# cvg/nice-slam

Hardware: NVIDIA H100
Metric: rendered rays/sec (higher is better)
Workload: dtype f32

## Files before the change

### nice_slam_b200/csrc/nsb_tc.cuh

```cuda
#pragma once

namespace nsb {
namespace tc {

#ifdef NSB_PHASE_TIMING
__device__ long long g_phase[64];
__device__ long long g_phase_last;
#define NSB_PH(id) do { if (blockIdx.x == 0 && threadIdx.x == 0) { const long long c_ = clock64(); ::nsb::tc::g_phase[id] += c_ - ::nsb::tc::g_phase_last; ::nsb::tc::g_phase_last = c_; } } while (0)
#define NSB_PH_RESET() do { if (blockIdx.x == 0 && threadIdx.x == 0) ::nsb::tc::g_phase_last = clock64(); } while (0)
#else
#define NSB_PH(id) do { } while (0)
#define NSB_PH_RESET() do { } while (0)
#endif

constexpr int TM = 128;
constexpr int kThreads = 512;
constexpr int kCG = kThreads / TM;
constexpr int kCW = 32 / kCG;
constexpr int kKQ = kCW / 4;

__device__ __forceinline__ float to_tf32(float x) { return __uint_as_float(__float_as_uint(x) & 0xffffe000u); }

__device__ __forceinline__ int canon_q(int r, int kq, int K) { return ((r >> 3) * (K >> 2) + kq) * 32 + (r & 7) * 4; }

// ... 11 lines not shown
  d |= (uint64_t)((smem_u32(smem) >> 4) & 0x3FFF);
  d |= (uint64_t)((lbo_bytes >> 4) & 0x3FFF) << 16;
  d |= (uint64_t)((sbo_bytes >> 4) & 0x3FFF) << 32;
  return d;
}

constexpr int kAccCols = 256;
constexpr int kAccSlotsPerSm = 4;
constexpr int kAccMaxSm = 144;
__device__ float g_acc_pool[(size_t)kAccMaxSm * kAccSlotsPerSm * kAccCols * TM];
__device__ int g_acc_lock[kAccMaxSm * kAccSlotsPerSm];
__shared__ float* s_acc;
__device__ __forceinline__ uint32_t acc_acquire() {
  uint32_t smid;
  asm volatile("mov.u32 %0, %%smid;" : "=r"(smid));
  if (smid >= (uint32_t)kAccMaxSm) __trap();
  const long long t0 = clock64();
  for (;;) {
    for (int k = 0; k < kAccSlotsPerSm; k++) {
      const int s = (int)smid * kAccSlotsPerSm + k;
      if (atomicCAS(&g_acc_lock[s], 0, 1) == 0) {
        __threadfence();
        s_acc = g_acc_pool + (size_t)s * kAccCols * TM;
        return (uint32_t)s;
      }
    }
    if (clock64() - t0 > 4000000000ll) __trap();
  }
}
__device__ __forceinline__ void acc_release(uint32_t slot) { __threadfence(); atomicExch(&g_acc_lock[slot], 0); }
__device__ __forceinline__ const float* acc_col(uint32_t taddr) { return s_acc + (size_t)(taddr & 0xffffu) * TM + (taddr >> 16) + (threadIdx.x & 31); }

__device__ __forceinline__ void wg_fence() { asm volatile("wgmma.fence.sync.aligned;" ::: "memory"); }
__device__ __forceinline__ void wg_commit_wait() {
  asm volatile("wgmma.commit_group.sync.aligned;" ::: "memory");
  asm volatile("wgmma.wait_group.sync.aligned 0;" ::: "memory");
}
__device__ __forceinline__ void wg_commit() { asm volatile("wgmma.commit_group.sync.aligned;" ::: "memory"); }
__device__ __forceinline__ void wg_wait0() { asm volatile("wgmma.wait_group.sync.aligned 0;" ::: "memory"); }
template <int N>
__device__ __forceinline__ void wg_wait() { asm volatile("wgmma.wait_group.sync.aligned %0;" ::"n"(N) : "memory"); }
__device__ __forceinline__ void fence_acc(float (&d)[16]) {
#pragma unroll
  for (int e = 0; e < 16; e++) asm volatile("" : "+f"(d[e])::"memory");
}
#define NSB_WG_D16 "+f"(d[0]), "+f"(d[1]), "+f"(d[2]), "+f"(d[3]), "+f"(d[4]), "+f"(d[5]), "+f"(d[6]), "+f"(d[7]), \
                   "+f"(d[8]), "+f"(d[9]), "+f"(d[10]), "+f"(d[11]), "+f"(d[12]), "+f"(d[13]), "+f"(d[14]), "+f"(d[15])
__device__ __forceinline__ void wgmma_tf32_n32(float (&d)[16], uint64_t da, uint64_t db) {
  asm volatile("{\n\t.reg .pred p;\n\tsetp.ne.b32 p, 1, 0;\n\t"
               "wgmma.mma_async.sync.aligned.m64n32k8.f32.tf32.tf32 "
               "{%0,%1,%2,%3,%4,%5,%6,%7,%8,%9,%10,%11,%12,%13,%14,%15}, %16, %17, p, 1, 1;\n\t}"
               : NSB_WG_D16 : "l"(da), "l"(db));
}
__device__ __forceinline__ void wgmma_f16_n32(float (&d)[16], uint64_t da, uint64_t db) {
  asm volatile("{\n\t.reg .pred p;\n\tsetp.ne.b32 p, 1, 0;\n\t"
               "wgmma.mma_async.sync.aligned.m64n32k16.f32.f16.f16 "
               "{%0,%1,%2,%3,%4,%5,%6,%7,%8,%9,%10,%11,%12,%13,%14,%15}, %16, %17, p, 1, 1, 0, 0;\n\t}"
               : NSB_WG_D16 : "l"(da), "l"(db));
}
#define NSB_WG_D32 "+f"(d0[0]), "+f"(d0[1]), "+f"(d0[2]), "+f"(d0[3]), "+f"(d0[4]), "+f"(d0[5]), "+f"(d0[6]), "+f"(d0[7]), \
                   "+f"(d0[8]), "+f"(d0[9]), "+f"(d0[10]), "+f"(d0[11]), "+f"(d0[12]), "+f"(d0[13]), "+f"(d0[14]), "+f"(d0[15]), \
                   "+f"(d1[0]), "+f"(d1[1]), "+f"(d1[2]), "+f"(d1[3]), "+f"(d1[4]), "+f"(d1[5]), "+f"(d1[6]), "+f"(d1[7]), \
                   "+f"(d1[8]), "+f"(d1[9]), "+f"(d1[10]), "+f"(d1[11]), "+f"(d1[12]), "+f"(d1[13]), "+f"(d1[14]), "+f"(d1[15])
#define NSB_WG_R32 "{%0,%1,%2,%3,%4,%5,%6,%7,%8,%9,%10,%11,%12,%13,%14,%15,%16,%17,%18,%19,%20,%21,%22,%23,%24,%25,%26,%27,%28,%29,%30,%31}"
__device__ __forceinline__ void wgmma_tf32_n64(float (&d0)[16], float (&d1)[16], uint64_t da, uint64_t db) {
  asm volatile("{\n\t.reg .pred p;\n\tsetp.ne.b32 p, 1, 0;\n\t"
               "wgmma.mma_async.sync.aligned.m64n64k8.f32.tf32.tf32 " NSB_WG_R32 ", %32, %33, p, 1, 1;\n\t}"
               : NSB_WG_D32 : "l"(da), "l"(db));
}
__device__ __forceinline__ void wgmma_f16_n64(float (&d0)[16], float (&d1)[16], uint64_t da, uint64_t db) {
  asm volatile("{\n\t.reg .pred p;\n\tsetp.ne.b32 p, 1, 0;\n\t"
               "wgmma.mma_async.sync.aligned.m64n64k16.f32.f16.f16 " NSB_WG_R32 ", %32, %33, p, 1, 1, 0, 0;\n\t}"
               : NSB_WG_D32 : "l"(da), "l"(db));
}
__device__ __forceinline__ void frag_rc(int e, int& r, int& c) {
  const int l = threadIdx.x & 31, w = (threadIdx.x >> 5) & 3;
  r = 16 * w + (l >> 2) + 8 * ((e >> 1) & 1);
  c = 8 * (e >> 2) + 2 * (l & 3) + (e & 1);
}

template <bool H16>
__device__ __forceinline__ void wg_mma(uint32_t dcol, uint64_t ah, uint64_t al, uint32_t sboA, uint64_t bh, uint64_t bl, uint32_t sboB,
                                       int N, int ksteps, uint32_t acc) {
  const int wg = threadIdx.x >> 7, npairs = blockDim.x >> 8;
  const int rbase = 64 * (wg & 1);
  const uint64_t aoff = (uint64_t)((8u * sboA * (uint32_t)(wg & 1)) >> 4);
  for (int c = wg >> 1; c < (N >> 5); c += npairs) {
    float* base = s_acc + (size_t)(dcol + 32 * c) * TM + rbase;
    float d[16];
#pragma unroll
    for (int e = 0; e < 16; e++) { int r, cc; frag_rc(e, r, cc); d[e] = acc ? base[cc * TM + r] : 0.0f; }
    const uint64_t boff = (uint64_t)((4u * sboB * (uint32_t)c) >> 4);
    wg_fence();
#pragma unroll 1
    for (int ks = 0; ks < ksteps; ks++) {
      const uint64_t o = 16u * (uint64_t)ks;
      if (H16) {
        wgmma_f16_n32(d, al + aoff + o, bh + boff + o); wgmma_f16_n32(d, ah + aoff + o, bl + boff + o); wgmma_f16_n32(d, ah + aoff + o, bh + boff + o);
      } else {
        wgmma_tf32_n32(d, al + aoff + o, bh + boff + o); wgmma_tf32_n32(d, ah + aoff + o, bl + boff + o); wgmma_tf32_n32(d, ah + aoff + o, bh + boff + o);
      }
    }
    wg_commit_wait();
#pragma unroll
    for (int e = 0; e < 16; e++) { int r, cc; frag_rc(e, r, cc); base[cc * TM + r] = d[e]; }
  }
}
__device__ __forceinline__ void mbar_arrive1(uint64_t* bar) { asm volatile("mbarrier.arrive.shared::cta.b64 _, [%0];" ::"r"(smem_u32(bar)) : "memory"); }
__device__ __forceinline__ void group_done(uint64_t* bar) {
  __syncthreads();
  if (threadIdx.x == 0) mbar_arrive1(bar);
}
__device__ __forceinline__ void mma_3x(uint32_t d_tmem, const float* a_hi, const float* a_lo, int KA, int ka0,
                                       const float* b_hi, const float* b_lo, int KB, int kb0, int kcount, int N, uint32_t& acc) {
  const uint32_t sboA = (uint32_t)(KA >> 2) * 128u, sboB = (uint32_t)(KB >> 2) * 128u;
  const uint64_t ah0 = make_desc(a_hi + (ka0 >> 2) * 32, 128u, sboA), al0 = make_desc(a_lo + (ka0 >> 2) * 32, 128u, sboA);
  const uint64_t bh0 = make_desc(b_hi + (kb0 >> 2) * 32, 128u, sboB), bl0 = make_desc(b_lo + (kb0 >> 2) * 32, 128u, sboB);
  wg_mma<false>(d_tmem & 0xffffu, ah0, al0, sboA, bh0, bl0, sboB, N, kcount, acc);
  acc = 1u;
}
__device__ __forceinline__ void publish_operands() { fence_proxy_async(); __syncthreads(); }

__device__ __forceinline__ void acc_ld8(uint32_t taddr, float (&v)[8]) {
  const float* p = acc_col(taddr);
#pragma unroll
  for (int j = 0; j < 8; j++) v[j] = p[j * TM];
}
static_assert(kCW == 8, "epilogues read 8 accumulator columns per thread");

struct TcSmem {
  float* x;
// ... 355 lines not shown
```

### nice_slam_b200/csrc/nsb_tile.cuh

```cuda
#pragma once

namespace nsb {
namespace tl {

using tc::TM;
constexpr int kThreads = 256;
constexpr int kEpiThreads = kThreads;
constexpr int kCG = 2, kCW = 16, kKQ = 4;
constexpr int kSlots = 4;
constexpr int kSlotFloatsFwd = 2560;
constexpr int kSlotFloatsBwd = 2048;
constexpr int kABufFloats = 2 * TM * 32;
constexpr int kMaxTileRays = 18;
constexpr int kMinSamples = 8;
constexpr long long kWaitCycles = 4000000000ll;

enum { B_FULL = 0, B_EMPTY = 4, B_HDR = 8, B_AREADY = 10, B_DONE = 12, kNumBars = 14 };

__device__ __forceinline__ bool mbar_try(uint64_t* bar, uint32_t parity) {
  uint32_t ok;
  asm volatile("{\n\t.reg .pred p;\n\tmbarrier.try_wait.parity.shared::cta.b64 p, [%1], %2;\n\tselp.b32 %0, 1, 0, p;\n\t}"
               : "=r"(ok) : "r"(smem_u32(bar)), "r"(parity) : "memory");
  return ok != 0;
}
// ... 95 lines not shown
  uint32_t issued;
  uint32_t g;
};
__device__ __forceinline__ void issuer_wait_operands(Issuer& I, const TileSmem& t, int b, uint32_t parity) {
  uint64_t* bar = t.bars + B_AREADY + b;
  const long long t0 = clock64();
  while (!mbar_test(bar, parity)) {
    if (threadIdx.x == 0) loader_top_up(I.L, t, I.issued);
    if (clock64() - t0 > kWaitCycles) __trap();
  }
}
__device__ __forceinline__ const float* issuer_unit(Issuer& I, const TileSmem& t, uint32_t k = 0) {
  if (threadIdx.x == 0) {
    loader_top_up(I.L, t, I.issued);
    while (I.L.loaded <= I.issued + k) loader_refill(I.L, t, I.issued);
  }
  const uint32_t u = I.issued + k;
  const int slot = u & (kSlots - 1);
  mbar_wait_b(t.bars + B_FULL + slot, (u >> 2) & 1u);
  return t.ring + slot * t.slot_floats;
}
__device__ __forceinline__ const float* issued_unit(const Issuer& I, const TileSmem& t, uint32_t k) { return t.ring + ((I.issued + k) & (kSlots - 1)) * t.slot_floats; }

__device__ __forceinline__ uint32_t cvt_h2(float lo_elem, float hi_elem) {
  uint32_t r;
  asm("cvt.rn.satfinite.f16x2.f32 %0, %1, %2;" : "=r"(r) : "f"(hi_elem), "f"(lo_elem));
  return r;
}
__device__ __forceinline__ void split_h2(float x, float y, uint32_t& h, uint32_t& l) {
  h = cvt_h2(x, y);
  const float2 f = __half22float2(*reinterpret_cast<const __half2*>(&h));
  l = cvt_h2(x - f.x, y - f.y);
}
__device__ __forceinline__ void put4_h(float* tile, int r, int kq, const float4 v) {
  unsigned char* hi = reinterpret_cast<unsigned char*>(tile) + (((r >> 3) * 4 + (kq >> 1)) * 128 + (r & 7) * 16 + (kq & 1) * 8);
  uint2 h, l;
  split_h2(v.x, v.y, h.x, l.x); split_h2(v.z, v.w, h.y, l.y);
  *reinterpret_cast<uint2*>(hi) = h;
  *reinterpret_cast<uint2*>(hi + TM * 32 * 2) = l;
}
__device__ __forceinline__ void put16_h(float* tile, int r, int cg, const float (&v)[kCW]) {
#pragma unroll
  for (int c = 0; c < 2; c++) {
    unsigned char* hi = reinterpret_cast<unsigned char*>(tile) + (((r >> 3) * 4 + 2 * cg + c) * 128 + (r & 7) * 16);
    uint4 h, l;
    split_h2(v[8 * c], v[8 * c + 1], h.x, l.x); split_h2(v[8 * c + 2], v[8 * c + 3], h.y, l.y);
    split_h2(v[8 * c + 4], v[8 * c + 5], h.z, l.z); split_h2(v[8 * c + 6], v[8 * c + 7], h.w, l.w);
    *reinterpret_cast<uint4*>(hi) = h;
    *reinterpret_cast<uint4*>(hi + TM * 32 * 2) = l;
  }
}
struct RowsDesc { uint64_t ah, al, bh, bl; };
template <bool H16>
__device__ __forceinline__ RowsDesc rows_desc(const float* a, int ka0, const float* b, int N, int KB, int c) {
  const uint32_t g = (threadIdx.x >> 7) & 1u;
  const int esz = H16 ? 2 : 4, kcm = H16 ? 8 : 4;
  const uint32_t sbo_a = (32u / kcm) * 128u, sbo_b = (uint32_t)(KB / kcm) * 128u;
  RowsDesc r;
  r.ah = tc::make_desc(a + (ka0 / kcm) * 32, 128u, sbo_a) + (uint64_t)((8u * sbo_a * g) >> 4);
  r.bh = tc::make_desc(b, 128u, sbo_b) + (uint64_t)((4u * sbo_b * (uint32_t)c) >> 4);
  r.al = r.ah + (uint64_t)((TM * 32 * esz) >> 4); r.bl = r.bh + (uint64_t)((N * KB * esz) >> 4);
  return r;
}
template <bool H16, int ksteps>
__device__ __forceinline__ void mma_rows(float (&d)[16], const float* a, int ka0, const float* b, int N, int KB, int c) {
  const RowsDesc r = rows_desc<H16>(a, ka0, b, N, KB, c);
#pragma unroll
  for (int ks = 0; ks < ksteps; ks++) {
    const uint64_t o = 16u * (uint64_t)ks;
    if (H16) { tc::wgmma_f16_n32(d, r.al + o, r.bh + o); tc::wgmma_f16_n32(d, r.ah + o, r.bl + o); tc::wgmma_f16_n32(d, r.ah + o, r.bh + o); }
    else { tc::wgmma_tf32_n32(d, r.al + o, r.bh + o); tc::wgmma_tf32_n32(d, r.ah + o, r.bl + o); tc::wgmma_tf32_n32(d, r.ah + o, r.bh + o); }
  }
}
template <bool H16, int ksteps>
__device__ __forceinline__ void mma_rows64(float (&d0)[16], float (&d1)[16], const float* a, int ka0, const float* b, int N, int KB, int c) {
  const RowsDesc r = rows_desc<H16>(a, ka0, b, N, KB, c);
#pragma unroll
  for (int ks = 0; ks < ksteps; ks++) {
    const uint64_t o = 16u * (uint64_t)ks;
    if (H16) { tc::wgmma_f16_n64(d0, d1, r.al + o, r.bh + o); tc::wgmma_f16_n64(d0, d1, r.ah + o, r.bl + o); tc::wgmma_f16_n64(d0, d1, r.ah + o, r.bh + o); }
    else { tc::wgmma_tf32_n64(d0, d1, r.al + o, r.bh + o); tc::wgmma_tf32_n64(d0, d1, r.ah + o, r.bl + o); tc::wgmma_tf32_n64(d0, d1, r.ah + o, r.bh + o); }
  }
}
__device__ __forceinline__ void arrive_units(const TileSmem& t, uint32_t first, uint32_t count, uint64_t* done = nullptr) {
  if ((threadIdx.x & 127) == 0) {
    for (uint32_t k = 0; k < count; k++) mbar_arrive(t.bars + B_EMPTY + ((first + k) & (kSlots - 1)));
    if (done != nullptr) mbar_arrive(done);
  }
}
__device__ __forceinline__ void release_units(Issuer& I, const TileSmem& t, uint32_t count, uint64_t* done = nullptr) {
  arrive_units(t, I.issued, count, done);
  I.issued += count;
}
__device__ __forceinline__ void wg_bar_sync() {
  if (threadIdx.x >> 7) asm volatile("bar.sync 2, 128;" ::: "memory");
  else asm volatile("bar.sync 1, 128;" ::: "memory");
}
__device__ __forceinline__ void zero16(float (&d)[16]) {
#pragma unroll
  for (int e = 0; e < 16; e++) d[e] = 0.0f;
}
__device__ __forceinline__ void zero16_opaque(float (&d)[16]) {
#pragma unroll
  for (int e = 0; e < 16; e++) asm volatile("mov.b32 %0, 0;" : "=f"(d[e])::"memory");
}
__device__ __forceinline__ void put2(float* hi, int r, int c, float a, float b) {
  float* hp = hi + tc::canon_q(r, c >> 2, 32) + (c & 3);
  const float h0 = tc::to_tf32(a), h1 = tc::to_tf32(b);
  *reinterpret_cast<float2*>(hp) = make_float2(h0, h1);
  *reinterpret_cast<float2*>(hp + TM * 32) = make_float2(a - h0, b - h1);
}

__device__ __forceinline__ void publish(const TileSmem& t, int b) {
  fence_proxy_async();
  __syncwarp();
  if ((threadIdx.x & 31) == 0) mbar_arrive(t.bars + B_AREADY + b);
}
__device__ __forceinline__ void wait_group(const TileSmem& t, uint32_t m) {
  mbar_wait_b(t.bars + B_DONE + (m & 1u), (m >> 1) & 1u);
}

struct GatherPass {
  float4 v[8];
  float w[8];
// ... 81 lines not shown
#pragma unroll
  for (int k = 0; k < 4; k++) p[k] = make_float4(d[4 * k], d[4 * k + 1], d[4 * k + 2], d[4 * k + 3]);
}
template <bool H16, bool kAccumulate>
__device__ __forceinline__ void issue_fc(Issuer& I, const TileSmem& t, float (&d1)[16], float (&d3)[16]) {
  constexpr int nu = H16 ? 2 : 4;
  const int b = I.g & 1;
  issuer_wait_operands(I, t, b, (I.g >> 1) & 1u);
  NSB_PH(5);
#pragma unroll 1
  for (int u = 0; u < nu; u++) issuer_unit(I, t, u);
  NSB_PH(11);
#pragma unroll
  for (int c = 0; c < 5; c += 2) {
    const bool pair = c < 4;
    if (kAccumulate) { ld_frag(d2_frag(c), d1); if (pair) ld_frag(d2_frag(c + 1), d3); }
    else { zero16_opaque(d1); if (pair) zero16_opaque(d3); }
    tc::wg_fence();
#pragma unroll
    for (int u = 0; u < nu; u++) {
      if (pair) mma_rows64<H16, 1>(d1, d3, t.a[b], H16 ? 16 * u : 8 * u, issued_unit(I, t, u), 160, H16 ? 16 : 8, c);
      else mma_rows<H16, 1>(d1, t.a[b], H16 ? 16 * u : 8 * u, issued_unit(I, t, u), 160, H16 ? 16 : 8, c);
    }
    tc::wg_commit(); tc::wg_wait0(); tc::fence_acc(d1);
    st_frag(d2_frag(c), d1);
    if (pair) { tc::fence_acc(d3); st_frag(d2_frag(c + 1), d3); }
  }
  release_units(I, t, nu, t.bars + B_DONE + b);
  I.g++;
}
template <bool H16 = false>
__device__ __forceinline__ void issue_l0(Issuer& I, const TileSmem& t, float (&d1)[16], float (&d3)[16]) {
  constexpr int nu = H16 ? 1 : 2;
  const int b = I.g & 1;
  issuer_wait_operands(I, t, b, (I.g >> 1) & 1u);
  NSB_PH(10);
#pragma unroll 1
  for (int u = 0; u < nu; u++) issuer_unit(I, t, u);
  tc::wg_fence();
#pragma unroll
  for (int u = 0; u < nu; u++) mma_rows64<H16, 2>(d1, d3, t.a[b], 16 * u, issued_unit(I, t, u), 64, H16 ? 32 : 16, 0);
  tc::wg_commit();
  I.issued += nu;
  I.g++;
}
template <bool H16 = false>
__device__ __forceinline__ void release_l0(const Issuer& I, const TileSmem& t, uint32_t back, uint32_t count) {
  constexpr uint32_t nu = H16 ? 1 : 2;
  for (uint32_t j = back; j > back - count; j--) arrive_units(t, I.issued - j * nu, nu, t.bars + B_DONE + ((I.g - j) & 1u));
}
template <bool H16 = false>
__device__ __forceinline__ void issue_h(Issuer& I, const TileSmem& t, float (&d1)[16], const float (&d3)[16], const float* hbuf, int i) {
  const float* w = issuer_unit(I, t);
  if (i == 3) {
#pragma unroll
    for (int e = 0; e < 16; e++) d1[e] = d3[e];
  } else {
    zero16(d1);
  }
  tc::wg_fence();
  mma_rows<H16, H16 ? 2 : 4>(d1, hbuf, 0, w, 32, 32, 0);
  tc::wg_commit();
}

template <bool H16 = false>
__device__ __forceinline__ void epi_forward(const KParams& P, const TileSmem& t, Issuer& I, int lv, const PointGeom& G, uint32_t& n, int hb, uint32_t hdr_parity,
                                            float (&out)[4], uint32_t* __restrict__ masks, float* __restrict__ acts, int npts) {
  const int row = threadIdx.x & (TM - 1), cg = threadIdx.x >> 7, warp = threadIdx.x >> 5, lane = threadIdx.x & 31;
  const bool xyz = lv != 0;
  const int cd = op_cd(lv), no = lv == 3 ? 4 : 1;
  const float* hdr = t.hdr + hb * kHdrFloats;
  float d1[16], d3[16];
  if (xyz) {
    for (int half = 0; half < cd / 32; half++) {
      if (n >= 2) wait_group(t, n - 2);
      if (threadIdx.x == 0) loader_top_up(I.L, t, I.issued);
      gather_tile<H16>(P.in.grid[half == 0 ? lv : 1], t.a[n & 1], G.xn, warp, lane);
      NSB_PH(1);
      publish(t, n & 1); n++;
      if (half == 0) issue_fc<H16, false>(I, t, d1, d3); else issue_fc<H16, true>(I, t, d1, d3);
      NSB_PH(2);
    }
    mbar_wait_b(t.bars + B_HDR + hb, hdr_parity);
    zero16_opaque(d1); zero16_opaque(d3);
#pragma unroll
    for (int blk = 0; blk < 3; blk++) {
      if (n >= 2) wait_group(t, n - 2);
      if (threadIdx.x == 0) loader_top_up(I.L, t, I.issued);
      NSB_PH(6);
      embed_tile<H16>(t.a[n & 1], hdr + 464, G.pf, row, cg, blk);
      NSB_PH(3);
      publish(t, n & 1); n++;
      issue_l0<H16>(I, t, d1, d3);
      if (blk == 1) { tc::wg_wait<1>(); release_l0<H16>(I, t, 2, 1); }
      NSB_PH(4);
    }
  } else {
    if (n >= 2) wait_group(t, n - 2);
    gather_tile<H16>(P.in.grid[0], t.a[n & 1], G.xnc, warp, lane);
    publish(t, n & 1); n++;
    zero16_opaque(d1); zero16_opaque(d3);
    issue_l0<H16>(I, t, d1, d3);
    mbar_wait_b(t.bars + B_HDR + hb, hdr_parity);
  }
  tc::wg_wait0(); tc::fence_acc(d1); tc::fence_acc(d3);
  release_l0<H16>(I, t, xyz ? 2 : 1, xyz ? 2 : 1);
  st_frag(d2_frag(5), d3);
  float* hbuf = t.a[n & 1];
  const int wg = threadIdx.x >> 7, q = lane & 3;
  const int r0 = 64 * wg + 16 * (warp & 3) + (lane >> 2);
  float v2[16];
  if (xyz) ld_frag(d2_frag(0), v2);
#pragma unroll 1
  for (int i = 0; i < 5; i++) {
    if (threadIdx.x == 0) loader_top_up(I.L, t, I.issued);
    NSB_PH(7);
    uint32_t m0 = 0, m1 = 0;
#pragma unroll
    for (int e = 0; e < 16; e++) {
      const int c = 8 * (e >> 2) + 2 * q + (e & 1);
      const float u = d1[e] + hdr[i * 32 + c];
      const uint32_t bit = u > 0.0f ? 1u << (8 * (e >> 2) + (e & 1)) : 0u;
      if (e & 2) m1 |= bit; else m0 |= bit;
      float h = u > 0.0f ? u : 0.0f;
      if (xyz) h += v2[e] + hdr[160 + i * 32 + c];
      d1[e] = h;
    }
    if (masks != nullptr) {
      m0 <<= 2 * q; m1 <<= 2 * q;
      m0 |= __shfl_xor_sync(0xffffffffu, m0, 1); m1 |= __shfl_xor_sync(0xffffffffu, m1, 1);
      m0 |= __shfl_xor_sync(0xffffffffu, m0, 2); m1 |= __shfl_xor_sync(0xffffffffu, m1, 2);
      if (q == 0 && r0 < npts) masks[(size_t)r0 * 15 + i] = m0;
      if (q == 1 && r0 + 8 < npts) masks[(size_t)(r0 + 8) * 15 + i] = m1;
    }
    if (acts != nullptr) {
#pragma unroll
      for (int e = 0; e < 16; e += 2) {
        const int r = r0 + 8 * ((e >> 1) & 1), c = 8 * (e >> 2) + 2 * q;
        if (r < npts) __stcg(reinterpret_cast<float2*>(acts + (size_t)r * 160 + i * 32 + c), make_float2(d1[e], d1[e + 1]));
      }
    }
    if (i == 4) break;
    if (i == 2) ld_frag(d2_frag(5), d3);
#pragma unroll
    for (int e = 0; e < 16; e += 2) {
      const int r = r0 + 8 * ((e >> 1) & 1), c = 8 * (e >> 2) + 2 * q;
      if (H16) {
        unsigned char* hp = reinterpret_cast<unsigned char*>(hbuf) + (((r >> 3) * 4 + (c >> 3)) * 128 + (r & 7) * 16 + (c & 7) * 2);
        uint32_t hh, ll;
        split_h2(d1[e], d1[e + 1], hh, ll);
        *reinterpret_cast<uint32_t*>(hp) = hh;
        *reinterpret_cast<uint32_t*>(hp + TM * 32 * 2) = ll;
      } else {
        put2(hbuf, r, c, d1[e], d1[e + 1]);
      }
    }
    NSB_PH(8);
    fence_proxy_async();
    wg_bar_sync();
    issue_h<H16>(I, t, d1, d3, hbuf, i + 1);
    NSB_PH(9);
    if (xyz) ld_frag(d2_frag(i + 1), v2);
    tc::wg_wait0(); tc::fence_acc(d1); release_units(I, t, 1);
  }
  NSB_PH(8);
  float s0[4], s1[4];
#pragma unroll
  for (int o = 0; o < 4; o++) {
    s0[o] = s1[o] = 0.0f;
    if (o < no) {
#pragma unroll
      for (int e = 0; e < 16; e++) {
        const float w = hdr[336 + o * 32 + 8 * (e >> 2) + 2 * q + (e & 1)];
        if (e & 2) s1[o] = fmaf(d1[e], w, s1[o]); else s0[o] = fmaf(d1[e], w, s0[o]);
      }
    }
    s0[o] += __shfl_xor_sync(0xffffffffu, s0[o], 1); s1[o] += __shfl_xor_sync(0xffffffffu, s1[o], 1);
    s0[o] += __shfl_xor_sync(0xffffffffu, s0[o], 2); s1[o] += __shfl_xor_sync(0xffffffffu, s1[o], 2);
  }
  constexpr int kWgHiFloats = 64 * 32 / (H16 ? 2 : 1);
  auto part = [&](int r) { return reinterpret_cast<float4*>(hbuf + (r >> 6) * kWgHiFloats + (r & 63) * 4); };
  if (q == 0) *part(r0) = make_float4(s0[0], s0[1], s0[2], s0[3]);
  if (q == 1) *part(r0 + 8) = make_float4(s1[0], s1[1], s1[2], s1[3]);
  epi_sync();
  {
    const float4 v = *part(row);
    out[0] = hdr[320] + v.x; out[1] = hdr[321] + v.y; out[2] = hdr[322] + v.z; out[3] = hdr[323] + v.w;
  }
  epi_sync();
  NSB_PH(12);
}

constexpr int kMnTile = TM * 32;
constexpr size_t kWgBytes = (size_t)6 * kMnTile * 4;
constexpr int kWgALo = 2 * kMnTile, kWgBLo = kMnTile;
struct WgSmem { float* du; float* g; float* b; float* dpk; };
__host__ __device__ __forceinline__ int acts_slot(int mask, int lv) { return (mask >> lv) & 1 ? __builtin_popcount(mask & ((1 << lv) - 1)) : -1; }
struct WgDec { int o_W0, o_W1, o_W2, o_W3E, o_W3H, o_W4, o_WC, PC, o_WO, no, o_b, o_bc, o_bo; };
template <int LV>
__device__ __forceinline__ WgDec wg_dec() {
  using D = Dec<LV>;
  return WgDec{D::o_W0, D::o_W1, D::o_W2, D::o_W3E, D::o_W3H, D::o_W4, D::o_WC, D::PC, D::o_WO, D::NO, D::o_b, D::o_bc, D::o_bo};
}
static_assert(Dec<0>::PH == Dec<3>::PH && Dec<1>::PH == Dec<3>::PH && Dec<2>::PH == Dec<3>::PH, "shared hidden pitch of the WG decoders");
static_assert(Dec<1>::PF == Dec<3>::PF && Dec<2>::PF == Dec<3>::PF && Dec<1>::o_B == Dec<3>::o_B && Dec<2>::o_B == Dec<3>::o_B,
              "shared first-input pitch and embedding block of the xyz WG decoders");
static_assert(Dec<1>::o_WO == Dec<3>::o_WO && Dec<1>::o_bo == Dec<3>::o_bo && Dec<1>::TOTAL == Dec<3>::TOTAL, "middle decoder = colour layout");
__device__ __forceinline__ void split4(const float4 v, float4& h, float4& l) {
  h = make_float4(tc::to_tf32(v.x), tc::to_tf32(v.y), tc::to_tf32(v.z), tc::to_tf32(v.w));
  l = make_float4(v.x - h.x, v.y - h.y, v.z - h.z, v.w - h.w);
}
__device__ __forceinline__ int kt_idx(int f, int p) { return ((f >> 3) * (TM / 4) + (p >> 2)) * 32 + (f & 7) * 4 + (p & 3); }
// ... 63 lines not shown
      }
    }
  }
  __syncthreads();
}
__device__ __forceinline__ float warp_colsum16(const float (&v)[kCW], int lane) {
  float a[8];
#pragma unroll
  for (int j = 0; j < 8; j++) { const float give = (lane & 16) ? v[j] : v[j + 8], keep = (lane & 16) ? v[j + 8] : v[j]; a[j] = keep + __shfl_xor_sync(0xffffffffu, give, 16); }
  float b[4];
#pragma unroll
  for (int j = 0; j < 4; j++) { const float give = (lane & 8) ? a[j] : a[j + 4], keep = (lane & 8) ? a[j + 4] : a[j]; b[j] = keep + __shfl_xor_sync(0xffffffffu, give, 8); }
  float c[2];
#pragma unroll
  for (int j = 0; j < 2; j++) { const float give = (lane & 4) ? b[j] : b[j + 2], keep = (lane & 4) ? b[j + 2] : b[j]; c[j] = keep + __shfl_xor_sync(0xffffffffu, give, 4); }
  const float give = (lane & 2) ? c[0] : c[1], keep = (lane & 2) ? c[1] : c[0];
  float d = keep + __shfl_xor_sync(0xffffffffu, give, 2);
  d += __shfl_xor_sync(0xffffffffu, d, 1);
  return d;
}
__device__ __forceinline__ int colsum_col(int lane) { return ((lane >> 4) & 1) * 8 + ((lane >> 3) & 1) * 4 + ((lane >> 2) & 1) * 2 + ((lane >> 1) & 1); }
__device__ __forceinline__ float frag_colsum(const float (&v)[16], int lane) {
  float a[8];
#pragma unroll
  for (int j = 0; j < 8; j++) a[j] = v[4 * (j >> 1) + (j & 1)] + v[4 * (j >> 1) + (j & 1) + 2];
  float b[4];
#pragma unroll
  for (int j = 0; j < 4; j++) { const float give = (lane & 16) ? a[j] : a[j + 4], keep = (lane & 16) ? a[j + 4] : a[j]; b[j] = keep + __shfl_xor_sync(0xffffffffu, give, 16); }
  float c[2];
#pragma unroll
  for (int j = 0; j < 2; j++) { const float give = (lane & 8) ? b[j] : b[j + 2], keep = (lane & 8) ? b[j + 2] : b[j]; c[j] = keep + __shfl_xor_sync(0xffffffffu, give, 8); }
  const float give = (lane & 4) ? c[0] : c[1], keep = (lane & 4) ? c[1] : c[0];
  return keep + __shfl_xor_sync(0xffffffffu, give, 4);
}
__device__ __forceinline__ int frag_colsum_col(int lane) {
  const int j = ((lane >> 4) & 1) * 4 + ((lane >> 3) & 1) * 2 + ((lane >> 2) & 1);
  return 8 * (j >> 1) + 2 * (lane & 3) + (j & 1);
}

struct BwdExtra {
  double dp[TM * 3];
  double z[TM];
  float gocc[TM];
  float wgt[TM];
  float gc[kMaxTileRays * 3];
};
__device__ __forceinline__ void bwd_gout(const BwdExtra& X, int lv, int r, int npts, int off0, int S, float (&go)[4]) {
  go[0] = go[1] = go[2] = go[3] = 0.0f;
  if (r >= npts) return;
  if (lv == 3) { const float w = X.wgt[r]; const float* gc = X.gc + 3 * ((off0 + r) / S); go[0] = w * gc[0]; go[1] = w * gc[1]; go[2] = w * gc[2]; }
  else go[0] = X.gocc[r];
}

template <bool DC, int NDF, bool L0>
__device__ __forceinline__ void issue_bwd_layer_t(Issuer& I, const TileSmem& t, int ndc, float (&d1)[16], float (&dc)[16], float (&fa)[16]) {
  constexpr int ND1 = L0 ? 0 : 1, FMAX = L0 ? 2 : 1;
  constexpr int kWaves = NDF > FMAX ? (NDF + FMAX - 1) / FMAX : 1;
#pragma unroll
  for (int wave = 0; wave < kWaves; wave++) {
    const int f0 = wave * FMAX;
    const int nf = NDF - f0 < FMAX ? NDF - f0 : FMAX;
    const int k = wave == 0 ? ndc + ND1 : 0;
    const int nu = k + nf;
#pragma unroll 1
    for (int u = 0; u < nu; u++) issuer_unit(I, t, u);
    if (nf > 0) { if (L0) ld_frag(d2_frag(f0), fa); else zero16_opaque(fa); }
    if (nf > 1) ld_frag(d2_frag(f0 + 1), d1);
    if (wave == 0 && ND1) zero16_opaque(d1);
    tc::wg_fence();
    if (wave == 0) {
      if (DC) mma_rows<false, 4>(dc, t.a[0], 0, issued_unit(I, t, 0), 32, 32, 0);
      if (ND1) mma_rows<false, 4>(d1, t.a[1], 0, issued_unit(I, t, ndc), 32, 32, 0);
    }
    if (nf > 0) mma_rows<false, 4>(fa, t.a[1], 0, issued_unit(I, t, k), 32, 32, 0);
    if (nf > 1) mma_rows<false, 4>(d1, t.a[1], 0, issued_unit(I, t, k + 1), 32, 32, 0);
    tc::wg_commit(); tc::wg_wait0();
    tc::fence_acc(dc); tc::fence_acc(d1); tc::fence_acc(fa);
    if (nf > 0) st_frag(d2_frag(f0), fa);
    if (nf > 1) st_frag(d2_frag(f0 + 1), d1);
    release_units(I, t, nu);
  }
}
template <bool XYZ>
__device__ __forceinline__ void issue_bwd_layer_x(Issuer& I, const TileSmem& t, int ndc, int i, float (&d1)[16], float (&dc)[16], float (&fa)[16]) {
  constexpr int NDF = op_firstp(XYZ ? 1 : 0) / 32;
  if (XYZ && i == 4) zero16_opaque(dc);
  if (i == 3) issue_bwd_layer_t<XYZ, NDF, false>(I, t, ndc, d1, dc, fa);
  else if (i == 0) issue_bwd_layer_t<XYZ, NDF, true>(I, t, ndc, d1, dc, fa);
  else issue_bwd_layer_t<XYZ, 0, false>(I, t, ndc, d1, dc, fa);
}
__device__ __forceinline__ void issue_bwd_layer(Issuer& I, const TileSmem& t, int lv, int i, float (&d1)[16], float (&dc)[16], float (&fa)[16]) {
  if (lv != 0) issue_bwd_layer_x<true>(I, t, op_cd(lv) / 32, i, d1, dc, fa);
  else issue_bwd_layer_x<false>(I, t, 0, i, d1, dc, fa);
}

enum { kWgNone = 0, kWgXyz = 1, kWgCoarse = 2 };
__device__ __forceinline__ int bwd_dpe_off(int r) { return (r >> 6) * (64 * 32) + (r & 63) * 4; }
template <int WG>
__device__ __forceinline__ void epi_backward(const KParams& P, const TileSmem& t, Issuer& I, const BwdExtra& X, int lv, const PointGeom& G, int hb, uint32_t hdr_parity,
                                             const uint32_t* __restrict__ masks, int npts, int off0, long long gp0, WgSmem* w = nullptr, const float* acts_row = nullptr) {
  const int row = threadIdx.x & (TM - 1), cg = threadIdx.x >> 7, warp = threadIdx.x >> 5;
  const int lane = threadIdx.x & 31, q = lane & 3;
  const int r0 = 64 * (threadIdx.x >> 7) + 16 * (warp & 3) + (lane >> 2);
  const int S = P.S;
  constexpr bool kWg = WG != kWgNone;
  constexpr int PH = Dec<3>::PH, PF = WG == kWgCoarse ? Dec<0>::PF : Dec<3>::PF;
  const WgDec DW = WG == kWgCoarse ? wg_dec<0>() : lv == 2 ? wg_dec<2>() : wg_dec<3>();
  float creg[kCW], cmid[kCW];
  const bool xyz = WG == kWgCoarse ? false : lv != 0;
  const float* hdr = t.hdr + hb * kHdrFloats;
  uint32_t m01 = 0, m23 = 0, m4 = 0;
  {
    const uint32_t* w0 = masks + (size_t)(r0 < npts ? r0 : npts - 1) * 15;
    const uint32_t* w1 = masks + (size_t)(r0 + 8 < npts ? r0 + 8 : npts - 1) * 15;
#pragma unroll
    for (int i = 0; i < 5; i++) {
      const uint32_t v = ((w0[i] >> (2 * q)) & 0x03030303u) | (((w1[i] >> (2 * q)) & 0x03030303u) << 2);
      if (i == 4) m4 = v; else if (i & 2) m23 |= v << (4 * (i & 1)); else m01 |= v << (4 * (i & 1));
    }
  }
  mbar_wait_b(t.bars + B_HDR + hb, hdr_parity);
  float d1[16], dc[16], fa[16];
  {
    float go0[4], go1[4];
    bwd_gout(X, lv, r0, npts, off0, S, go0); bwd_gout(X, lv, r0 + 8, npts, off0, S, go1);
#pragma unroll
    for (int e = 0; e < 16; e++) {
      float v = 0.0f;
#pragma unroll
      for (int o = 0; o < 4; o++) v = fmaf(hdr[336 + o * 32 + 8 * (e >> 2) + 2 * q + (e & 1)], (e & 2) ? go1[o] : go0[o], v);
      d1[e] = v;
    }
  }
  if constexpr (kWg) {
    float g_out[4];
    bwd_gout(X, lv, row, npts, off0, S, g_out);
    gather_tile_kt(P.in.grid[lv], w->b, kWgBLo, WG == kWgCoarse ? G.xnc : G.xn, warp, lane);
    __syncthreads();
    get_kt16(w->b, kWgBLo, row, cg, creg);
    __syncthreads();
    if (lv == 2) {
      gather_tile_kt(P.in.grid[NSB_MIDDLE], w->b, kWgBLo, G.xn, warp, lane);
      __syncthreads();
      get_kt16(w->b, kWgBLo, row, cg, cmid);
      __syncthreads();
    }
    float go[kCW];
#pragma unroll
    for (int j = 0; j < kCW; j++) go[j] = (cg == 0 && j < 4) ? g_out[j] : 0.0f;
    put_kt16(w->du, kWgALo, row, cg, go);
    float h4[kCW];
#pragma unroll
    for (int k = 0; k < kKQ; k++) {
      const float4 v = acts_row != nullptr ? __ldcg(reinterpret_cast<const float4*>(acts_row + 4 * 32 + 4 * k)) : make_float4(0.f, 0.f, 0.f, 0.f);
      h4[4 * k] = v.x; h4[4 * k + 1] = v.y; h4[4 * k + 2] = v.z; h4[4 * k + 3] = v.w;
    }
    put_kt16(w->b, kWgBLo, row, cg, h4);
    wg_group(*w, 0, w->dpk + DW.o_WO, PH, DW.no);
    if (cg == 0) {
      const float sb = warp_colsum16(go, lane);
      const int col = colsum_col(lane);
      if ((lane & 1) == 0 && col < DW.no) atomicAdd(w->dpk + DW.o_bo + col, sb);
    }
  }
#pragma unroll 1
  for (int i = 4; i >= 0; i--) {
    const uint32_t m = (i == 4 ? m4 : (i & 2) ? m23 : m01) >> (4 * (i & 1));
    float du[16];
#pragma unroll
    for (int e = 0; e < 16; e++) du[e] = (m >> (8 * (e >> 2) + 2 * ((e >> 1) & 1) + (e & 1))) & 1u ? d1[e] : 0.0f;
#pragma unroll
    for (int e = 0; e < 16; e += 2) {
      const int r = r0 + 8 * ((e >> 1) & 1), c = 8 * (e >> 2) + 2 * q;
      if (xyz) put2(t.a[0], r, c, d1[e], d1[e + 1]);
      put2(t.a[1], r, c, du[e], du[e + 1]);
    }
    if constexpr (kWg) {
#pragma unroll
      for (int e = 0; e < 16; e++) {
        const int r = r0 + 8 * ((e >> 1) & 1), c = 8 * (e >> 2) + 2 * q + (e & 1);
        put_kt1(w->du, kWgALo, c, r, du[e]);
        if constexpr (WG != kWgCoarse) put_kt1(w->g, kWgALo, c, r, d1[e]);
      }
      const float sb = frag_colsum(du, lane);
      float sc = 0.0f;
      if constexpr (WG != kWgCoarse) sc = frag_colsum(d1, lane);
      const int col = frag_colsum_col(lane);
      atomicAdd(w->dpk + DW.o_b + 32 * i + col, sb);
      if constexpr (WG != kWgCoarse) atomicAdd(w->dpk + DW.o_bc + 32 * i + col, sc);
    }
    fence_proxy_async();
    wg_bar_sync();
    NSB_PH(22);
    issue_bwd_layer(I, t, WG == kWgCoarse ? 0 : lv, i, d1, dc, fa);
    if (threadIdx.x == 0) loader_top_up(I.L, t, I.issued);
    NSB_PH(23);
    if constexpr (kWg) {
      if (i >= 1) {
        float xr[kCW];
#pragma unroll
        for (int k = 0; k < kKQ; k++) {
          const float4 v = acts_row != nullptr ? __ldcg(reinterpret_cast<const float4*>(acts_row + (i - 1) * 32 + 4 * k)) : make_float4(0.f, 0.f, 0.f, 0.f);
          xr[4 * k] = v.x; xr[4 * k + 1] = v.y; xr[4 * k + 2] = v.z; xr[4 * k + 3] = v.w;
        }
        put_kt16(w->b, kWgBLo, row, cg, xr);
        const int o_wh = i == 1 ? DW.o_W1 : i == 2 ? DW.o_W2 : i == 3 ? DW.o_W3H : DW.o_W4;
        wg_group(*w, 0, w->dpk + o_wh, PH, 32);
      }
      if constexpr (WG != kWgCoarse) {
        put_kt16(w->b, kWgBLo, row, cg, creg);
        wg_group(*w, 1, w->dpk + DW.o_WC + 32 * i * DW.PC, DW.PC, 32);
        if (lv == 2) {
          put_kt16(w->b, kWgBLo, row, cg, cmid);
          wg_group(*w, 1, w->dpk + DW.o_WC + 32 * i * DW.PC + 32, DW.PC, 32);
        }
      }
      if (i == 3 || i == 0) {
        if constexpr (WG != kWgCoarse) {
          const float* B = hdr + 464;
          for (int blk = 0; blk < 3; blk++) {
            float e[kCW];
#pragma unroll
            for (int j = 0; j < kCW; j++) {
              const int f = 32 * blk + kCW * cg + j;
              float x = G.pf[0] * B[f]; x = fmaf(G.pf[1], B[kEmbPad + f], x); x = fmaf(G.pf[2], B[2 * kEmbPad + f], x);
              e[j] = f < kEmb ? __sinf(reduce_2pi(x)) : 0.0f;
            }
            put_kt16(w->b, kWgBLo, row, cg, e);
            wg_group(*w, 0, w->dpk + (i == 0 ? DW.o_W0 : DW.o_W3E) + 32 * blk, PF, 32);
          }
        } else {
          put_kt16(w->b, kWgBLo, row, cg, creg);
          wg_group(*w, 0, w->dpk + (i == 0 ? DW.o_W0 : DW.o_W3E), PF, 32);
        }
      }
      NSB_PH(24);
    }
  }
  if (!xyz) ld_frag(d2_frag(0), dc);
#pragma unroll
  for (int e = 0; e < 16; e += 2) {
    const int r = r0 + 8 * ((e >> 1) & 1), c = 8 * (e >> 2) + 2 * q;
    *reinterpret_cast<float2*>(t.a[0] + r * 32 + c) = make_float2(dc[e], dc[e + 1]);
  }
  float dpe0[3] = {0.0f, 0.0f, 0.0f}, dpe1[3] = {0.0f, 0.0f, 0.0f};
  if (xyz) {
    const float* B = hdr + 464;
// ... 374 lines not shown
```

Before: 1.258 million.

## Feed hidden-layer MMA A operand from registers instead of shared memory

Adds a register-sourced wgmma variant for TF32 and a shuffle-based conversion of the accumulator fragment into the A-operand layout, split into hi/lo TF32 parts. The forward hidden layers and the backward hidden layers without DF chunks now feed activations straight from registers. This skips the shared-memory staging stores, the async-proxy fence and the warpgroup barrier on those paths. In exchange it adds shuffles and register pressure, and the register-fragment permutation must be exactly right for correctness.

```diff
diff --git a/nice_slam_b200/csrc/nsb_tc.cuh b/nice_slam_b200/csrc/nsb_tc.cuh
--- a/nice_slam_b200/csrc/nsb_tc.cuh
+++ b/nice_slam_b200/csrc/nsb_tc.cuh
@@ -87,6 +87,12 @@
                "{%0,%1,%2,%3,%4,%5,%6,%7,%8,%9,%10,%11,%12,%13,%14,%15}, %16, %17, p, 1, 1;\n\t}"
                : NSB_WG_D16 : "l"(da), "l"(db));
 }
+__device__ __forceinline__ void wgmma_tf32_n32_rs(float (&d)[16], const uint32_t (&a)[4], uint64_t db) {
+  asm volatile("{\n\t.reg .pred p;\n\tsetp.ne.b32 p, 1, 0;\n\t"
+               "wgmma.mma_async.sync.aligned.m64n32k8.f32.tf32.tf32 "
+               "{%0,%1,%2,%3,%4,%5,%6,%7,%8,%9,%10,%11,%12,%13,%14,%15}, {%16,%17,%18,%19}, %20, p, 1, 1;\n\t}"
+               : NSB_WG_D16 : "r"(a[0]), "r"(a[1]), "r"(a[2]), "r"(a[3]), "l"(db));
+}
 __device__ __forceinline__ void wgmma_f16_n32(float (&d)[16], uint64_t da, uint64_t db) {
   asm volatile("{\n\t.reg .pred p;\n\tsetp.ne.b32 p, 1, 0;\n\t"
                "wgmma.mma_async.sync.aligned.m64n32k16.f32.f16.f16 "
@@ -112,6 +118,24 @@
   const int l = threadIdx.x & 31, w = (threadIdx.x >> 5) & 3;
   r = 16 * w + (l >> 2) + 8 * ((e >> 1) & 1);
   c = 8 * (e >> 2) + 2 * (l & 3) + (e & 1);
+}
+__device__ __forceinline__ void frag_a_tf32(const float (&d)[16], uint32_t (&ah)[16], uint32_t (&al)[16]) {
+  const int lane = threadIdx.x & 31, q = lane & 3, quad = lane & ~3;
+  const int src1 = quad | ((q & 1) << 1) | (q >> 1), src2 = quad | (((q & 1) ^ 1) << 1) | (q >> 1);
+  const bool upper = (q >> 1) != 0;
+#pragma unroll
+  for (int j = 0; j < 4; j++) {
+#pragma unroll
+    for (int h = 0; h < 2; h++) {
+      const float x0 = d[4 * j + 2 * h], x1 = d[4 * j + 2 * h + 1];
+      const float v1 = __shfl_sync(0xffffffffu, upper ? x1 : x0, src1);
+      const float v2 = __shfl_sync(0xffffffffu, upper ? x0 : x1, src2);
+      const float cq = (q & 1) ? v2 : v1, cq4 = (q & 1) ? v1 : v2;
+      const float hq = to_tf32(cq), hq4 = to_tf32(cq4);
+      ah[4 * j + h] = __float_as_uint(hq); al[4 * j + h] = __float_as_uint(cq - hq);
+      ah[4 * j + 2 + h] = __float_as_uint(hq4); al[4 * j + 2 + h] = __float_as_uint(cq4 - hq4);
+    }
+  }
 }
 
 template <bool H16>
diff --git a/nice_slam_b200/csrc/nsb_tile.cuh b/nice_slam_b200/csrc/nsb_tile.cuh
--- a/nice_slam_b200/csrc/nsb_tile.cuh
+++ b/nice_slam_b200/csrc/nsb_tile.cuh
@@ -171,14 +171,21 @@
 }
 struct RowsDesc { uint64_t ah, al, bh, bl; };
 template <bool H16>
+__device__ __forceinline__ void b_desc(const float* b, int N, int KB, int c, uint64_t& bh, uint64_t& bl) {
+  const int esz = H16 ? 2 : 4, kcm = H16 ? 8 : 4;
+  const uint32_t sbo_b = (uint32_t)(KB / kcm) * 128u;
+  bh = tc::make_desc(b, 128u, sbo_b) + (uint64_t)((4u * sbo_b * (uint32_t)c) >> 4);
+  bl = bh + (uint64_t)((N * KB * esz) >> 4);
+}
+template <bool H16>
 __device__ __forceinline__ RowsDesc rows_desc(const float* a, int ka0, const float* b, int N, int KB, int c) {
   const uint32_t g = (threadIdx.x >> 7) & 1u;
   const int esz = H16 ? 2 : 4, kcm = H16 ? 8 : 4;
-  const uint32_t sbo_a = (32u / kcm) * 128u, sbo_b = (uint32_t)(KB / kcm) * 128u;
+  const uint32_t sbo_a = (32u / kcm) * 128u;
   RowsDesc r;
   r.ah = tc::make_desc(a + (ka0 / kcm) * 32, 128u, sbo_a) + (uint64_t)((8u * sbo_a * g) >> 4);
-  r.bh = tc::make_desc(b, 128u, sbo_b) + (uint64_t)((4u * sbo_b * (uint32_t)c) >> 4);
-  r.al = r.ah + (uint64_t)((TM * 32 * esz) >> 4); r.bl = r.bh + (uint64_t)((N * KB * esz) >> 4);
+  r.al = r.ah + (uint64_t)((TM * 32 * esz) >> 4);
+  b_desc<H16>(b, N, KB, c, r.bh, r.bl);
   return r;
 }
 template <bool H16, int ksteps>
@@ -189,6 +196,18 @@
     const uint64_t o = 16u * (uint64_t)ks;
     if (H16) { tc::wgmma_f16_n32(d, r.al + o, r.bh + o); tc::wgmma_f16_n32(d, r.ah + o, r.bl + o); tc::wgmma_f16_n32(d, r.ah + o, r.bh + o); }
     else { tc::wgmma_tf32_n32(d, r.al + o, r.bh + o); tc::wgmma_tf32_n32(d, r.ah + o, r.bl + o); tc::wgmma_tf32_n32(d, r.ah + o, r.bh + o); }
+  }
+}
+template <int ksteps>
+__device__ __forceinline__ void mma_rows_rs(float (&d)[16], const uint32_t (&ah)[4 * ksteps], const uint32_t (&al)[4 * ksteps], const float* b, int N, int KB, int c) {
+  uint64_t bh, bl;
+  b_desc<false>(b, N, KB, c, bh, bl);
+#pragma unroll
+  for (int ks = 0; ks < ksteps; ks++) {
+    const uint64_t o = 16u * (uint64_t)ks;
+    const uint32_t (&h)[4] = *reinterpret_cast<const uint32_t (*)[4]>(ah + 4 * ks);
+    const uint32_t (&l)[4] = *reinterpret_cast<const uint32_t (*)[4]>(al + 4 * ks);
+    tc::wgmma_tf32_n32_rs(d, l, bh + o); tc::wgmma_tf32_n32_rs(d, h, bl + o); tc::wgmma_tf32_n32_rs(d, h, bh + o);
   }
 }
 template <bool H16, int ksteps>
@@ -376,6 +395,8 @@
 template <bool H16 = false>
 __device__ __forceinline__ void issue_h(Issuer& I, const TileSmem& t, float (&d1)[16], const float (&d3)[16], const float* hbuf, int i) {
   const float* w = issuer_unit(I, t);
+  uint32_t ah[16], al[16];
+  if constexpr (!H16) tc::frag_a_tf32(d1, ah, al);
   if (i == 3) {
 #pragma unroll
     for (int e = 0; e < 16; e++) d1[e] = d3[e];
@@ -383,7 +404,8 @@
     zero16(d1);
   }
   tc::wg_fence();
-  mma_rows<H16, H16 ? 2 : 4>(d1, hbuf, 0, w, 32, 32, 0);
+  if constexpr (H16) mma_rows<true, 2>(d1, hbuf, 0, w, 32, 32, 0);
+  else mma_rows_rs<4>(d1, ah, al, w, 32, 32, 0);
   tc::wg_commit();
 }
 
@@ -466,22 +488,22 @@
     }
     if (i == 4) break;
     if (i == 2) ld_frag(d2_frag(5), d3);
-#pragma unroll
-    for (int e = 0; e < 16; e += 2) {
-      const int r = r0 + 8 * ((e >> 1) & 1), c = 8 * (e >> 2) + 2 * q;
-      if (H16) {
+    if constexpr (H16) {
+#pragma unroll
+      for (int e = 0; e < 16; e += 2) {
+        const int r = r0 + 8 * ((e >> 1) & 1), c = 8 * (e >> 2) + 2 * q;
         unsigned char* hp = reinterpret_cast<unsigned char*>(hbuf) + (((r >> 3) * 4 + (c >> 3)) * 128 + (r & 7) * 16 + (c & 7) * 2);
         uint32_t hh, ll;
         split_h2(d1[e], d1[e + 1], hh, ll);
         *reinterpret_cast<uint32_t*>(hp) = hh;
         *reinterpret_cast<uint32_t*>(hp + TM * 32 * 2) = ll;
-      } else {
-        put2(hbuf, r, c, d1[e], d1[e + 1]);
       }
-    }
-    NSB_PH(8);
-    fence_proxy_async();
-    wg_bar_sync();
+      NSB_PH(8);
+      fence_proxy_async();
+      wg_bar_sync();
+    } else {
+      NSB_PH(8);
+    }
     issue_h<H16>(I, t, d1, d3, hbuf, i + 1);
     NSB_PH(9);
     if (xyz) ld_frag(d2_frag(i + 1), v2);
@@ -651,8 +673,9 @@
   else go[0] = X.gocc[r];
 }
 
-template <bool DC, int NDF, bool L0>
-__device__ __forceinline__ void issue_bwd_layer_t(Issuer& I, const TileSmem& t, int ndc, float (&d1)[16], float (&dc)[16], float (&fa)[16]) {
+template <bool DC, int NDF, bool L0, bool RS>
+__device__ __forceinline__ void issue_bwd_layer_t(Issuer& I, const TileSmem& t, int ndc, const float (&du)[16], float (&d1)[16], float (&dc)[16], float (&fa)[16]) {
+  static_assert(!RS || (NDF == 0 && !L0), "DU from registers only in the hidden layers without DF chunks");
   constexpr int ND1 = L0 ? 0 : 1, FMAX = L0 ? 2 : 1;
   constexpr int kWaves = NDF > FMAX ? (NDF + FMAX - 1) / FMAX : 1;
 #pragma unroll
@@ -663,13 +686,15 @@
     const int nu = k + nf;
 #pragma unroll 1
     for (int u = 0; u < nu; u++) issuer_unit(I, t, u);
+    uint32_t uh[16], ul[16];
+    if (RS) tc::frag_a_tf32(du, uh, ul);
     if (nf > 0) { if (L0) ld_frag(d2_frag(f0), fa); else zero16_opaque(fa); }
     if (nf > 1) ld_frag(d2_frag(f0 + 1), d1);
     if (wave == 0 && ND1) zero16_opaque(d1);
     tc::wg_fence();
     if (wave == 0) {
       if (DC) mma_rows<false, 4>(dc, t.a[0], 0, issued_unit(I, t, 0), 32, 32, 0);
-      if (ND1) mma_rows<false, 4>(d1, t.a[1], 0, issued_unit(I, t, ndc), 32, 32, 0);
+      if (ND1) { if (RS) mma_rows_rs<4>(d1, uh, ul, issued_unit(I, t, ndc), 32, 32, 0); else mma_rows<false, 4>(d1, t.a[1], 0, issued_unit(I, t, ndc), 32, 32, 0); }
     }
     if (nf > 0) mma_rows<false, 4>(fa, t.a[1], 0, issued_unit(I, t, k), 32, 32, 0);
     if (nf > 1) mma_rows<false, 4>(d1, t.a[1], 0, issued_unit(I, t, k + 1), 32, 32, 0);
@@ -680,17 +705,19 @@
     release_units(I, t, nu);
   }
 }
-template <bool XYZ>
-__device__ __forceinline__ void issue_bwd_layer_x(Issuer& I, const TileSmem& t, int ndc, int i, float (&d1)[16], float (&dc)[16], float (&fa)[16]) {
+__device__ __forceinline__ bool bwd_du_regs(bool du_regs, int i) { return du_regs && i != 3 && i != 0; }
+template <bool XYZ, bool RS>
+__device__ __forceinline__ void issue_bwd_layer_x(Issuer& I, const TileSmem& t, int ndc, int i, const float (&du)[16], float (&d1)[16], float (&dc)[16], float (&fa)[16]) {
   constexpr int NDF = op_firstp(XYZ ? 1 : 0) / 32;
   if (XYZ && i == 4) zero16_opaque(dc);
-  if (i == 3) issue_bwd_layer_t<XYZ, NDF, false>(I, t, ndc, d1, dc, fa);
-  else if (i == 0) issue_bwd_layer_t<XYZ, NDF, true>(I, t, ndc, d1, dc, fa);
-  else issue_bwd_layer_t<XYZ, 0, false>(I, t, ndc, d1, dc, fa);
-}
-__device__ __forceinline__ void issue_bwd_layer(Issuer& I, const TileSmem& t, int lv, int i, float (&d1)[16], float (&dc)[16], float (&fa)[16]) {
-  if (lv != 0) issue_bwd_layer_x<true>(I, t, op_cd(lv) / 32, i, d1, dc, fa);
-  else issue_bwd_layer_x<false>(I, t, 0, i, d1, dc, fa);
+  if (i == 3) issue_bwd_layer_t<XYZ, NDF, false, false>(I, t, ndc, du, d1, dc, fa);
+  else if (i == 0) issue_bwd_layer_t<XYZ, NDF, true, false>(I, t, ndc, du, d1, dc, fa);
+  else issue_bwd_layer_t<XYZ, 0, false, RS>(I, t, ndc, du, d1, dc, fa);
+}
+template <bool RS>
+__device__ __forceinline__ void issue_bwd_layer(Issuer& I, const TileSmem& t, int lv, int i, const float (&du)[16], float (&d1)[16], float (&dc)[16], float (&fa)[16]) {
+  if (lv != 0) issue_bwd_layer_x<true, RS>(I, t, op_cd(lv) / 32, i, du, d1, dc, fa);
+  else issue_bwd_layer_x<false, RS>(I, t, 0, i, du, d1, dc, fa);
 }
 
 enum { kWgNone = 0, kWgXyz = 1, kWgCoarse = 2 };
@@ -703,6 +730,7 @@
   const int r0 = 64 * (threadIdx.x >> 7) + 16 * (warp & 3) + (lane >> 2);
   const int S = P.S;
   constexpr bool kWg = WG != kWgNone;
+  constexpr bool kDuRegs = WG != kWgXyz;
   constexpr int PH = Dec<3>::PH, PF = WG == kWgCoarse ? Dec<0>::PF : Dec<3>::PF;
   const WgDec DW = WG == kWgCoarse ? wg_dec<0>() : lv == 2 ? wg_dec<2>() : wg_dec<3>();
   float creg[kCW], cmid[kCW];
@@ -768,11 +796,12 @@
     float du[16];
 #pragma unroll
     for (int e = 0; e < 16; e++) du[e] = (m >> (8 * (e >> 2) + 2 * ((e >> 1) & 1) + (e & 1))) & 1u ? d1[e] : 0.0f;
+    const bool du_smem = !bwd_du_regs(kDuRegs, i);
 #pragma unroll
     for (int e = 0; e < 16; e += 2) {
       const int r = r0 + 8 * ((e >> 1) & 1), c = 8 * (e >> 2) + 2 * q;
       if (xyz) put2(t.a[0], r, c, d1[e], d1[e + 1]);
-      put2(t.a[1], r, c, du[e], du[e + 1]);
+      if (du_smem) put2(t.a[1], r, c, du[e], du[e + 1]);
     }
     if constexpr (kWg) {
 #pragma unroll
@@ -788,10 +817,12 @@
       atomicAdd(w->dpk + DW.o_b + 32 * i + col, sb);
       if constexpr (WG != kWgCoarse) atomicAdd(w->dpk + DW.o_bc + 32 * i + col, sc);
     }
-    fence_proxy_async();
-    wg_bar_sync();
+    if (xyz || du_smem) {
+      fence_proxy_async();
+      wg_bar_sync();
+    }
     NSB_PH(22);
-    issue_bwd_layer(I, t, WG == kWgCoarse ? 0 : lv, i, d1, dc, fa);
+    issue_bwd_layer<kDuRegs>(I, t, WG == kWgCoarse ? 0 : lv, i, du, d1, dc, fa);
     if (threadIdx.x == 0) loader_top_up(I.L, t, I.issued);
     NSB_PH(23);
     if constexpr (kWg) {
```

Result: faster. 1.286 million, median of 6 (+2.2%).
